# cv3vpl-lab/cylinder-pose-estimation

Hardware: AMD Instinct MI355X
Metric: frames/sec (grid-detect + cylinder fit) on 1920x1200 batch (higher is better)
Workload: dtype f64

## Files before the change

### cylinder-pose-estimation_amd/csrc/masks.hip

```cpp
#include "cpe_dev.h"

namespace cpe {

namespace {

struct W3 { unsigned long long a, b, c; };
template <int K> __device__ __forceinline__ W3 w3_up(const W3 &v, unsigned long long fill)
{
    W3 r;
    r.a = (v.a >> K) | (v.b << (64 - K));
    r.b = (v.b >> K) | (v.c << (64 - K));
    r.c = (v.c >> K) | (fill << (64 - K));
    return r;
}
template <int K> __device__ __forceinline__ W3 w3_down(const W3 &v, unsigned long long fill)
{
    W3 r;
    r.c = (v.c << K) | (v.b >> (64 - K));
    r.b = (v.b << K) | (v.a >> (64 - K));
    r.a = (v.a << K) | (fill >> (64 - K));
    return r;
}
__device__ __forceinline__ W3 w3_and(const W3 &x, const W3 &y) { return W3{x.a & y.a, x.b & y.b, x.c & y.c}; }
__device__ __forceinline__ W3 w3_or(const W3 &x, const W3 &y) { return W3{x.a | y.a, x.b | y.b, x.c | y.c}; }
template <bool IS_AND> __device__ __forceinline__ W3 w3_window20(const W3 &v)
{
    const unsigned long long f = IS_AND ? ~0ull : 0ull;
    auto op = [](const W3 &x, const W3 &y) { return IS_AND ? w3_and(x, y) : w3_or(x, y); };
    const W3 t1 = op(v, w3_up<1>(v, f));
    const W3 t2 = op(t1, w3_up<2>(t1, f));
    const W3 t4 = op(t2, w3_up<4>(t2, f));
    const W3 t8 = op(t4, w3_up<8>(t4, f));
    const W3 t20 = op(t8, w3_up<12>(t4, f));
    return w3_down<10>(t20, f);
}
__device__ __forceinline__ unsigned long long row_valid_word(int j, int w)
{
    const int x0 = j * 64;
    if (j < 0 || x0 >= w) return 0ull;
    return (x0 + 64 <= w) ? ~0ull : ((1ull << (w - x0)) - 1ull);
}
__device__ __forceinline__ unsigned long long bytes_of_bits8(unsigned bits)
{
    unsigned long long v = ((unsigned long long)(bits & 255u) * 0x0101010101010101ull) & 0x8040201008040201ull;
    v = ((v + 0x7f7f7f7f7f7f7f7full) & 0x8080808080808080ull) >> 7;
    return v * 255ull;
}

constexpr int OB_AP = 20;
template <int R>
__global__ __launch_bounds__(256) void k_open20_joints(const uint8_t *__restrict__ bin, int h, int w, int bands,
                                                       uint8_t *__restrict__ hm, uint8_t *__restrict__ vm,
                                                       uint8_t *__restrict__ jm, uint32_t *__restrict__ jbits,
                                                       unsigned long long *__restrict__ hb, unsigned long long *__restrict__ vb)
{
    constexpr int ROWS = R + 2 * OB_AP;
    extern __shared__ unsigned long long s_ob[];
    const int WW = (w + 63) >> 6;
    unsigned long long *buf0 = s_ob, *buf1 = s_ob + (size_t)ROWS * WW, *hbuf = s_ob + (size_t)2 * ROWS * WW;
    const int t = threadIdx.x;
    const int f = blockIdx.x / bands, band = blockIdx.x - f * bands;
    const int y0 = band * R;
    const size_t N = (size_t)h * w;
    const uint8_t *im = bin + f * N;
    const bool al8 = ((w & 7) == 0) && (((size_t)im & 7) == 0);
    {
        uint8_t *pk = reinterpret_cast<uint8_t *>(buf0);
        const int per_row = WW * 8;
        for (int i = t; i < ROWS * per_row; i += 256) {
            const int r = i / per_row, k = i - r * per_row;
            const int y = y0 - OB_AP + r, x0 = k * 8;
            unsigned bits = 255u;
            if (y >= 0 && y < h && x0 < w) {
                const uint8_t *q = im + (size_t)y * w + x0;
                if (al8) {
                    unsigned long long v = *reinterpret_cast<const unsigned long long *>(q);
                    v = (((v & 0x7f7f7f7f7f7f7f7full) + 0x7f7f7f7f7f7f7f7full) | v) & 0x8080808080808080ull;
                    bits = (unsigned)(((v >> 7) * 0x0102040810204080ull) >> 56);
                } else {
                    bits = 0;
                    for (int b = 0; b < 8; b++) bits |= ((x0 + b >= w) || q[b]) ? (1u << b) : 0u;
                }
            }
            pk[i] = (uint8_t)bits;
        }
    }
    __syncthreads();
    for (int i = t; i < R * WW; i += 256) {
        const int tr = i / WW, j = i - tr * WW;
        const unsigned long long *row = buf0 + (size_t)(tr + OB_AP) * WW;
        const W3 x{j > 0 ? row[j - 1] : ~0ull, row[j], j + 1 < WW ? row[j + 1] : ~0ull};
        const W3 v{row_valid_word(j - 1, w), row_valid_word(j, w), row_valid_word(j + 1, w)};
        const W3 e = w3_and(w3_window20<true>(x), v);
        hbuf[i] = w3_window20<false>(e).b & v.b;
    }
    __syncthreads();
    auto pass = [&](const unsigned long long *src, unsigned long long *dst, int step, bool is_and, const unsigned long long *src2) {
        const unsigned long long fill = is_and ? ~0ull : 0ull;
        for (int i = t; i < ROWS * WW; i += 256) {
            const int r = i / WW;
            const unsigned long long p = src[i];
            const unsigned long long q = (r + step < ROWS) ? src2[i + (size_t)step * WW] : fill;
            dst[i] = is_and ? (p & q) : (p | q);
        }
        __syncthreads();
    };
    pass(buf0, buf1, 1, true, buf0);
    pass(buf1, buf0, 2, true, buf1);
    pass(buf0, buf1, 4, true, buf0);
    pass(buf1, buf0, 8, true, buf1);
    for (int i = t; i < ROWS * WW; i += 256) {
        const int r = i / WW;
        const unsigned long long q = (r + 12 < ROWS) ? buf1[i + (size_t)12 * WW] : ~0ull;
        const int y = y0 - 10 + r;
        buf0[i] = (y >= 0 && y < h) ? (buf0[i] & q) : 0ull;
    }
    __syncthreads();
    pass(buf0, buf1, 1, false, buf0);
    pass(buf1, buf0, 2, false, buf1);
    pass(buf0, buf1, 4, false, buf0);
    pass(buf1, buf0, 8, false, buf1);
    {
        const int per_row = WW * 8;
        for (int i = t; hm && i < R * per_row; i += 256) {
            const int tr = i / per_row, k = i - tr * per_row;
            const int y = y0 + tr, x0 = k * 8;
            if (y >= h || x0 >= w) continue;
            const int j = k >> 3, sh = (k & 7) * 8;
            const size_t wi = (size_t)tr * WW + j;
            const unsigned long long d16 = buf0[wi] | ((tr + 12 < ROWS) ? buf1[wi + (size_t)12 * WW] : 0ull);
            const unsigned hb = (unsigned)(hbuf[wi] >> sh) & 255u;
            const unsigned vb = (unsigned)(d16 >> sh) & 255u;
            const size_t o = f * N + (size_t)y * w + x0;
            if (al8 && (((size_t)hm | (size_t)vm | (size_t)jm) & 7) == 0) {
                *reinterpret_cast<unsigned long long *>(hm + o) = bytes_of_bits8(hb);
                *reinterpret_cast<unsigned long long *>(vm + o) = bytes_of_bits8(vb);
                if (jm) *reinterpret_cast<unsigned long long *>(jm + o) = bytes_of_bits8(hb & vb);
            } else {
                for (int b = 0; b < 8 && x0 + b < w; b++) {
                    hm[o + b] = ((hb >> b) & 1u) ? 255 : 0;
                    vm[o + b] = ((vb >> b) & 1u) ? 255 : 0;
                    if (jm) jm[o + b] = (((hb & vb) >> b) & 1u) ? 255 : 0;
                }
            }
        }
        auto plane_word = [&](int tr, int j, bool hsel, bool vsel) {
            const size_t wi = (size_t)tr * WW + j;
            unsigned long long m = ~0ull;
            if (hsel) m &= hbuf[wi];
            if (vsel) m &= buf0[wi] | ((tr + 12 < ROWS) ? buf1[wi + (size_t)12 * WW] : 0ull);
            if (64 * j + 64 > w) m &= (1ull << (w - 64 * j)) - 1ull;
            return m;
        };
        store_plane_band(bit_plane(jbits, f, h, w), h, w, y0, R, t, [&](int tr, int j) { return plane_word(tr, j, true, true); });
        if (hb) {
            const size_t pw = bit_plane_words(h, w);
            store_plane_band(hb + f * pw, h, w, y0, R, t, [&](int tr, int j) { return plane_word(tr, j, true, false); });
            store_plane_band(vb + f * pw, h, w, y0, R, t, [&](int tr, int j) { return plane_word(tr, j, false, true); });
        }
    }
}

constexpr int RB_R = 64, RB_AP = 4, RB_ROWS = RB_R + 2 * RB_AP;
__global__ __launch_bounds__(256) void k_roi_base(const uint8_t *__restrict__ m, const uint8_t *__restrict__ cm,
                                                  const uint8_t *__restrict__ mc, int h, int w, int bands,
                                                  const FrameState *__restrict__ st, uint8_t *__restrict__ roi,
                                                  uint8_t *__restrict__ base, uint8_t *__restrict__ exp,
                                                  uint32_t *__restrict__ bbits, const unsigned long long *__restrict__ mb)
{
    extern __shared__ unsigned long long s_rb[];
    const int WW = (w + 63) >> 6;
    unsigned long long *buf0 = s_rb, *buf1 = s_rb + (size_t)RB_ROWS * WW, *mcb = s_rb + (size_t)2 * RB_ROWS * WW;
    const int t = threadIdx.x;
    const int f = blockIdx.x / bands, band = blockIdx.x - f * bands;
    const int y0 = band * RB_R;
    const size_t N = (size_t)h * w;
    const int *rc = st[f].rect;
    const int rx0 = rc[0], ry0 = rc[1], rx1 = rc[0] + rc[2] - 1, ry1 = rc[1] + rc[3] - 1;
    const bool al8 = ((w & 7) == 0) && ((((size_t)m | (size_t)cm | (size_t)mc | (size_t)roi | (size_t)base | (size_t)exp) & 7) == 0);
    const int per_row = WW * 8;
    auto store8 = [&](uint8_t *dst, size_t o, int x0, unsigned bits) {
        if (al8) *reinterpret_cast<unsigned long long *>(dst + o) = bytes_of_bits8(bits);
        else for (int b = 0; b < 8 && x0 + b < w; b++) dst[o + b] = ((bits >> b) & 1u) ? 255 : 0;
    };
    if (st[f].status == CPE_ST_NO_REGION || y0 > ry1 + RB_AP || y0 + RB_R - 1 < ry0 - RB_AP) {
        for (int i = t; i < RB_R * per_row; i += 256) {
            const int tr = i / per_row, k = i - tr * per_row;
            const int y = y0 + tr, x0 = k * 8;
            if (y >= h || x0 >= w) continue;
            const size_t o = f * N + (size_t)y * w + x0;
            if (roi) store8(roi, o, x0, 0u);
            store8(exp, o, x0, 0u);
            if (base) store8(base, o, x0, 0u);
        }
        store_plane_band(bit_plane(bbits, f, h, w), h, w, y0, RB_R, t, [](int, int) { return 0ull; });
        return;
    }
    {
        uint8_t *pk = reinterpret_cast<uint8_t *>(buf0), *pkc = reinterpret_cast<uint8_t *>(mcb);
        auto nonzero8 = [](unsigned long long v) {
            v = (((v & 0x7f7f7f7f7f7f7f7full) + 0x7f7f7f7f7f7f7f7full) | v) & 0x8080808080808080ull;
            return (unsigned)(((v >> 7) * 0x0102040810204080ull) >> 56);
        };
        const unsigned long long *mbf = mb ? mb + f * bit_plane_words(h, w) : nullptr;
        const int btc = bit_tile_cols(w);
        for (int i = t; i < RB_ROWS * per_row; i += 256) {
            const int r = i / per_row, k = i - r * per_row;
            const int y = y0 - RB_AP + r, x0 = k * 8;
            unsigned bits = 0u, cbits = 0u;
            if (y >= ry0 && y <= ry1 && y >= 0 && y < h && x0 < w && x0 + 7 >= rx0 && x0 <= rx1) {
                const size_t o = f * N + (size_t)y * w + x0;
                const unsigned mbits = mbf ? (unsigned)(mbf[bit_word(btc, y, k >> 3)] >> ((k & 7) * 8)) & 255u : 255u;
                if (al8) {
                    const unsigned long long vc = *reinterpret_cast<const unsigned long long *>(mc + o);
                    unsigned long long v = *reinterpret_cast<const unsigned long long *>(cm + o) & vc;
                    if (!mbf) v &= *reinterpret_cast<const unsigned long long *>(m + o);
                    bits = nonzero8(v) & mbits;
                    cbits = nonzero8(vc);
                } else {
                    for (int b = 0; b < 8 && x0 + b < w; b++) {
                        bits |= (((mbf ? 255 : m[o + b]) & cm[o + b]) & mc[o + b]) ? (1u << b) : 0u;
                        cbits |= mc[o + b] ? (1u << b) : 0u;
                    }
                    bits &= mbits;
                }
            }
            pk[i] = (uint8_t)bits;
            pkc[i] = (uint8_t)cbits;
        }
    }
    __syncthreads();
    auto pass = [&](const unsigned long long *src, unsigned long long *dst, bool dil) {
        const unsigned long long fill = dil ? 0ull : ~0ull;
        for (int i = t; i < RB_ROWS * WW; i += 256) {
            const int r = i / WW, j = i - r * WW;
            unsigned long long acc = fill;
#pragma unroll
            for (int dr = -1; dr <= 1; dr++) {
                const int rr = r + dr, y = y0 - RB_AP + rr;
                unsigned long long hres = fill;
                if (rr >= 0 && rr < RB_ROWS && y >= 0 && y < h) {
                    const unsigned long long *row = src + (size_t)rr * WW;
                    const unsigned long long va = row_valid_word(j - 1, w), vb = row_valid_word(j, w), vc = row_valid_word(j + 1, w);
                    unsigned long long xa = j > 0 ? row[j - 1] : 0ull, xb = row[j], xc = j + 1 < WW ? row[j + 1] : 0ull;
                    if (!dil) { xa |= ~va; xb |= ~vb; xc |= ~vc; }
                    const unsigned long long up = (xb >> 1) | (xc << 63), down = (xb << 1) | (xa >> 63);
                    hres = dil ? (xb | up | down) : (xb & up & down);
                }
                acc = dil ? (acc | hres) : (acc & hres);
            }
            const int y = y0 - RB_AP + r;
            dst[i] = (y >= 0 && y < h) ? (acc & row_valid_word(j, w)) : 0ull;
        }
        __syncthreads();
    };
    auto emit = [&](const unsigned long long *src, uint8_t *dst, uint8_t *dst2, const unsigned long long *and2) {
        for (int i = t; i < RB_R * per_row; i += 256) {
            const int tr = i / per_row, k = i - tr * per_row;
            const int y = y0 + tr, x0 = k * 8;
            if (y >= h || x0 >= w) continue;
            const size_t wi = (size_t)(tr + RB_AP) * WW + (k >> 3);
            const unsigned bits = (unsigned)(src[wi] >> ((k & 7) * 8)) & 255u;
            const size_t o = f * N + (size_t)y * w + x0;
            if (dst) store8(dst, o, x0, bits);
            if (dst2) store8(dst2, o, x0, bits & (unsigned)(and2[wi] >> ((k & 7) * 8)));
        }
    };
    pass(buf0, buf1, false);
    pass(buf1, buf0, true);
    if (roi) emit(buf0, roi, nullptr, nullptr);
    pass(buf0, buf1, true);
    pass(buf1, buf0, false);
    emit(buf0, base, exp, mcb);
    store_plane_band(bit_plane(bbits, f, h, w), h, w, y0, RB_R, t, [&](int tr, int j) { return buf0[(size_t)(tr + RB_AP) * WW + j]; });
}

__global__ __launch_bounds__(64) void k_joint_centroids(const uint32_t *__restrict__ jbits, int h, int w,
                                                        const int *__restrict__ roots, FrameState *__restrict__ st,
                                                        int *__restrict__ jtmp ,
                                                        const unsigned long long *__restrict__ outside, size_t plane_words)
{
    __shared__ unsigned long long s_win[BW_ROWS * 64];
    const int f = blockIdx.y;
    if (st[f].status != CPE_ST_OK) return;
    const int ncomp = min(st[f].n_roots_p, MAXROOTS);
    for (int k = blockIdx.x * 64 + threadIdx.x; k < ncomp; k += gridDim.x * 64) {
        const int root = roots[(size_t)f * MAXROOTS + k];
        if (!comp_is_external(outside + f * plane_words, w, root, 0)) continue;
        BitWin nz{bit_plane(jbits, f, h, w), w, h, s_win + threadIdx.x};
        StatVisitor sv;
        if (!trace_border(nz, root % w, root / w, false, sv, 4 * (w + h) + 65536)) { set_overflow(st[f], OVF_TRACE); continue; }
        sv.finish();
        double m00, m10, m01;
        moments_from_sums(sv.a00, sv.a10, sv.a01, m00, m10, m01);
        if (m00 == 0) continue;
        int cx = (int)(m10 / m00), cy = (int)(m01 / m00);
        atomicAdd(&st[f].n_joints_all, 1);
        const int *r = st[f].rect;
        if (!(r[0] <= cx && cx < r[0] + r[2] && r[1] <= cy && cy < r[1] + r[3])) continue;
        int q = atomicAdd(&st[f].n_joints, 1);
        if (q >= MAXJ) { set_overflow(st[f], OVF_JOINTS); continue; }
        int *o = jtmp + ((size_t)f * MAXJ + q) * 3;
        o[0] = cx; o[1] = cy; o[2] = root;
    }
}

__global__ __launch_bounds__(256) void k_joint_sort(FrameState *__restrict__ st, const int *__restrict__ jtmp,
                                                    int *__restrict__ joints )
{
    const int f = blockIdx.x;
    const int nj = min(st[f].n_joints, MAXJ);
    const int *src = jtmp + (size_t)f * MAXJ * 3;
    int *dst = joints + (size_t)f * MAXJ * 2;
    for (int i = threadIdx.x; i < nj; i += 256) {
        int ki = src[3 * i + 2], rank = 0;
        for (int j = 0; j < nj; j++) rank += (src[3 * j + 2] > ki) ? 1 : 0;
        dst[2 * rank] = src[3 * i];
        dst[2 * rank + 1] = src[3 * i + 1];
    }
    __syncthreads();
    if (threadIdx.x == 0) st[f].n_joints = nj;
}

struct Taps { int k[19]; int r; int shift; };

constexpr int BT_X = 64, BT_Y = 32;
constexpr int B7_R = 3, B7_IH = BT_Y + 2 * B7_R, B7_QW = (BT_X + 8) / 4;
constexpr int B7_LDS_WORDS = B7_IH * BT_X / 2;
static_assert(B7_IH * B7_QW <= B7_LDS_WORDS && BT_X == 64 && BT_Y == 32, "blur_tile's thread maps");
template <int R>
__device__ __forceinline__ void blur_tile(const uint8_t *__restrict__ im, int h, int w, int gx0, int gy0, const Taps &t,
                                          uint8_t *__restrict__ out, uint32_t *s_buf )
{
    static_assert(R == B7_R, "the 7 x 7 tile");
    constexpr int IH = B7_IH, QW = B7_QW, TASKS = IH * (BT_X / 8), PER = (TASKS + 255) / 256;
    const int tid = threadIdx.x;
    const int ax0 = gx0 - 4, ay0 = gy0 - R;
    if (ax0 >= 0 && ax0 + 4 * QW <= w && ay0 >= 0 && ay0 + IH <= h && (w & 3) == 0 && (((size_t)im) & 3) == 0) {
        for (int i = tid; i < IH * QW; i += 256) {
            const int ry = i / QW, q = i - ry * QW;
            s_buf[i] = *reinterpret_cast<const uint32_t *>(im + (size_t)(ay0 + ry) * w + ax0 + 4 * q);
        }
    } else {
        uint8_t *s_in8 = reinterpret_cast<uint8_t *>(s_buf);
        for (int i = tid; i < IH * QW * 4; i += 256) {
            const int ry = i / (4 * QW), b = i - ry * 4 * QW;
            s_in8[i] = im[(size_t)reflect101(ay0 + ry, h) * w + reflect101(ax0 + b, w)];
        }
    }
    __syncthreads();
    uint32_t d[PER][4];
#pragma unroll
    for (int u = 0; u < PER; u++) {
        const int it = tid + 256 * u;
        if (it < TASKS) {
            const int ry = it >> 3, c0 = (it & 7) * 8;
#pragma unroll
// ... 856 lines not shown
    __shared__ uint8_t s_in[IH * IW];
    __shared__ uint16_t s_h[IH * BT_X];
    const int tid = threadIdx.x;
    const int tiles = tiles_x * tiles_y;
    const int f = blockIdx.x / tiles, tt = blockIdx.x - f * tiles;
    const int gx0 = (tt % tiles_x) * BT_X, gy0 = (tt / tiles_x) * BT_Y;
    const size_t N = (size_t)h * w;
    const FrameState &S = st[f];
    if (S.status != CPE_ST_OK) return;
    int half = (int)(S.r0 / 5.0);
    if (half < 3) half = 3;
    if (half > 10) half = half + 5;
    half = max(half, (int)(S.r0 / 4.5));
    const int m = half + 1;
    if (gx0 > S.rect[0] + S.rect[2] + m || gx0 + BT_X < S.rect[0] - m || gy0 > S.rect[1] + S.rect[3] + m || gy0 + BT_Y < S.rect[1] - m)
        return;
    const uint8_t *im = bgr + f * N * 3;
    uint32_t ch[PER][3];
    for (int c = 0; c < 3; c++) {
        for (int i = tid; i < IH * IW; i += 256) {
            int ry = i / IW, rx = i - ry * IW;
            s_in[i] = im[((size_t)reflect101(gy0 - R + ry, h) * w + reflect101(gx0 - R + rx, w)) * 3 + c];
        }
        __syncthreads();
        for (int i = tid; i < IH * BT_X; i += 256) {
            int ry = i / BT_X, rx = i - ry * BT_X;
            const uint8_t *p = &s_in[ry * IW + rx];
            int sacc = 0;
#pragma unroll
            for (int j = 0; j <= 2 * R; j++) sacc += t.k[j] * p[j];
            s_h[i] = (uint16_t)sacc;
        }
        __syncthreads();
#pragma unroll
        for (int q = 0; q < PER; q++) {
            const int i = tid + q * 256;
            int ry = i / BT_X, rx = i - ry * BT_X;
            const uint16_t *p = &s_h[ry * BT_X + rx];
            int sacc = 0;
#pragma unroll
            for (int j = 0; j <= 2 * R; j++) sacc += t.k[j] * (int)p[j * BT_X];
            ch[q][c] = (uint32_t)((sacc + (1 << (t.shift - 1))) >> t.shift);
        }
        __syncthreads();
    }
#pragma unroll
    for (int q = 0; q < PER; q++) {
        const int i = tid + q * 256;
        int ry = i / BT_X, rx = i - ry * BT_X;
        if (gy0 + ry < h && gx0 + rx < w)
            dst[f * N + (size_t)(gy0 + ry) * w + gx0 + rx] = (uint8_t)((ch[q][0] * 3735u + ch[q][1] * 19235u + ch[q][2] * 9798u + 16384u) >> 15);
    }
}

int blur7_bgr(const uint8_t *bgr, int n, int h, int w, const FrameState *st, uint8_t *dst, hipStream_t s)
{
    Taps t7 = {{2, 7, 14, 18, 14, 7, 2}, 3, 12};
    CPE_LAUNCH_BEGIN();
    const int tiles_x = (w + BT_X - 1) / BT_X, tiles_y = (h + BT_Y - 1) / BT_Y;
    CPE_KLAUNCH(k_blur7_bgr, dim3((unsigned)(n * tiles_x * tiles_y)), dim3(256), 0, s, bgr, h, w, tiles_x, tiles_y, t7, st, dst);
    CPE_CHECK_LAUNCH("blur7_bgr");
    return CPE_OK;
}

int blur7_u8(const uint8_t *src, int n, int h, int w, const FrameState *st, uint8_t *dst, hipStream_t s)
{
    Taps t7 = {{2, 7, 14, 18, 14, 7, 2}, 3, 12};
    CPE_LAUNCH_BEGIN();
    const int tiles_x = (w + BT_X - 1) / BT_X, tiles_y = (h + BT_Y - 1) / BT_Y;
    CPE_KLAUNCH((k_blur_fused<3>), dim3((unsigned)(n * tiles_x * tiles_y)), dim3(256), 0, s, src, h, w, tiles_x, tiles_y, t7,
                st, dst);
    CPE_CHECK_LAUNCH("blur7_u8");
    return CPE_OK;
}

int joints_mask_stage(int n, int h, int w, const MaskBuffers &B, FrameState *st, hipStream_t s)
{
    CPE_LAUNCH_BEGIN();
    const bool as_bits = line_masks_as_bits(B, w);
    CPE_CHECK_ARG(!as_bits || 2 * bit_plane_words(h, w) * 8 <= (size_t)h * w, "joints_mask_stage: frame too small for its line-mask planes");
    unsigned long long *hb = as_bits ? line_mask_bits(B, 0, n, h, w) : nullptr, *vb = as_bits ? line_mask_bits(B, 1, n, h, w) : nullptr;
    uint8_t *hm = as_bits && B.skip_debug ? nullptr : B.hmask, *vm = as_bits && B.skip_debug ? nullptr : B.vmask;
    uint8_t *jm = as_bits ? nullptr : B.joints_mask;
    {
        const int WW = (w + 63) / 64;
        const size_t lds64 = (size_t)(2 * (64 + 2 * OB_AP) + 64) * WW * 8, lds32 = (size_t)(2 * (32 + 2 * OB_AP) + 32) * WW * 8;
        CPE_CHECK_HIP(hipFuncSetAttribute(reinterpret_cast<const void *>(&k_open20_joints<64>), hipFuncAttributeMaxDynamicSharedMemorySize, 160 * 1024));
        CPE_CHECK_HIP(hipFuncSetAttribute(reinterpret_cast<const void *>(&k_open20_joints<32>), hipFuncAttributeMaxDynamicSharedMemorySize, 160 * 1024));
        if (lds64 <= 96 * 1024) {
            const int bands = (h + 63) / 64;
            CPE_KLAUNCH(k_open20_joints<64>, dim3((unsigned)(n * bands)), dim3(256), lds64, s, (const uint8_t *)B.binary, h, w, bands,
                        hm, vm, jm, B.jbits, hb, vb);
        } else {
            CPE_CHECK_ARG(lds32 <= 160 * 1024, "joints_mask_stage: frame too wide (%d columns)", w);
            const int bands = (h + 31) / 32;
            CPE_KLAUNCH(k_open20_joints<32>, dim3((unsigned)(n * bands)), dim3(256), lds32, s, (const uint8_t *)B.binary, h, w, bands,
                        hm, vm, jm, B.jbits, hb, vb);
        }
    }
    CPE_CHECK_LAUNCH("joints_mask_stage");
    int rc;
    if ((rc = ccl_components(B.joints_mask, B.jbits, n, h, w, 0, WIN_FRAME, B.lab_p, B.roots_p, ROOTS_JOINTS, st, s)) != CPE_OK) return rc;
    const size_t fl_words = (size_t)h * ((w + 63) / 64);
    return outside_flood(B.joints_mask, n, h, w, st, WIN_FRAME, B.fl_j, B.fl_j + (size_t)n * fl_words, fl_words, s, B.jbits);
}

int spot_stage(const uint8_t *gray, int n, int h, int w, const MaskBuffers &B, FrameState *st, hipStream_t s, int planar)
{
    const size_t total = (size_t)h * w * n;
    int rc;
    CPE_LAUNCH_BEGIN();
    Taps t19 = {{1, 1, 3, 5, 10, 15, 20, 27, 30, 32, 30, 27, 20, 15, 10, 5, 3, 1, 1}, 9, 16};
    {
        const int tiles_x = (w + BT_X - 1) / BT_X, tiles_y = (h + BT_Y - 1) / BT_Y;
        CPE_CHECK_ARG(tiles_x <= 128 && (size_t)tiles_x * tiles_y <= (size_t)MAXROOTS * sizeof(int), "spot_stage: frame too large");
        uint8_t *flags = reinterpret_cast<uint8_t *>(B.roots_s);
        const size_t fstride = (size_t)MAXROOTS * sizeof(int);
        CPE_KLAUNCH(k_spot_scan, dim3((unsigned)(n * tiles_y)), dim3(256), 0, s, gray, h, w, tiles_x, tiles_y, st, flags, fstride);
        CPE_KLAUNCH(k_blur19_spot, dim3((unsigned)(n * tiles_y)), dim3(256), 0, s, gray, h, w, tiles_x, tiles_y, t19,
                    (const uint8_t *)flags, fstride, B.g19);
    }
    if ((rc = ccl_components(B.g19, nullptr, n, h, w, 240, WIN_SPOT, B.lab_s, B.roots_s, ROOTS_SPOT, st, s)) != CPE_OK) return rc;
    CPE_KLAUNCH(k_spot_area, dim3(4, n), dim3(64), 0, s, B.g19, h, w, B.roots_s, st, B.best_s);
    (void)hipMemsetAsync(B.cm, 255, total, s);
    CPE_KLAUNCH(k_spot_ellipse, dim3(n), dim3(64), 0, s, B.g19, n, h, w, B.best_s, st, B.verts, B.cm, planar);
    CPE_CHECK_LAUNCH("spot_stage");
    return CPE_OK;
}

int masks_stage(const uint8_t *gray, int n, int h, int w, const MaskBuffers &B, FrameState *st, hipStream_t s,
                const RegionSide *side, int planar, hipStream_t sj)
{
    int rc;
    CPE_LAUNCH_BEGIN();
    CPE_KLAUNCH(k_masks_reset, dim3((n + 63) / 64), dim3(64), 0, s, st, n);
    const size_t fl_words = bit_plane_words(h, w);
    auto fl_plane = [&](int k) { return bit_plane(B.bits, (size_t)(2 + k) * n, h, w); };
    const bool jside = side && sj != s;
    if (jside) { (void)hipEventRecord(side->clahe_done, s); (void)hipStreamWaitEvent(sj, side->clahe_done, 0); }
    {
        hipStream_t q = jside ? sj : s;
        CPE_KLAUNCH(k_joint_centroids, dim3(frame_waves(n, 16, MAXROOTS / 64), n), dim3(64), 0, q, (const uint32_t *)B.jbits, h, w, B.roots_p, st, B.jtmp,
                    (const unsigned long long *)(B.fl_j + (size_t)n * h * ((w + 63) / 64)), (size_t)h * ((w + 63) / 64));
        CPE_KLAUNCH(k_joint_sort, dim3(n), dim3(256), 0, q, st, B.jtmp, B.joints);
    }
    const int rb_bands = (h + RB_R - 1) / RB_R;
    const size_t rb_lds = (size_t)3 * RB_ROWS * ((w + 63) / 64) * 8;
    CPE_CHECK_ARG(rb_lds <= 160 * 1024, "masks_stage: frame too wide (%d columns)", w);
    CPE_CHECK_HIP(hipFuncSetAttribute(reinterpret_cast<const void *>(&k_roi_base), hipFuncAttributeMaxDynamicSharedMemorySize, 160 * 1024));
    if (side) { (void)hipEventRecord(side->clahe_done, s); (void)hipStreamWaitEvent(side->s, side->clahe_done, 0); }
    for (int which = 0; which < 2; which++) {
        hipStream_t q = (which && side) ? side->s : s;
        const bool as_bits = line_masks_as_bits(B, w);
        const uint8_t *lm = as_bits ? nullptr : (which ? B.vmask : B.hmask);
        const unsigned long long *lmb = as_bits ? line_mask_bits(B, which, n, h, w) : nullptr;
        uint8_t *roi = as_bits && B.skip_debug ? nullptr : (which ? B.roi_v : B.roi_h);
        uint8_t *exp = which ? B.exp_v : B.exp_h;
        int *lab = which ? B.lab_s : B.lab, *roots = which ? B.roots_s : B.roots;
        const RootList list = which ? ROOTS_SPOT : ROOTS_MAIN;
        uint32_t *bits = reinterpret_cast<uint32_t *>(bit_plane(B.bits, which ? (size_t)n : 0, h, w));
        SegRec *segs = B.segs + (size_t)which * n * MAXSEG;
        uint8_t *base = ccl_components_reads_bits(bits, w, lab) ? nullptr : (which ? B.base_v : B.base_h);
        CPE_KLAUNCH(k_roi_base, dim3((unsigned)(n * rb_bands)), dim3(256), rb_lds, q, lm, (const uint8_t *)B.cm, (const uint8_t *)B.mc,
                    h, w, rb_bands, (const FrameState *)st, roi, base, exp, bits, lmb);
        if ((rc = ccl_components(base, bits, n, h, w, 0, WIN_REGION, lab, roots, list, st, q)) != CPE_OK) return rc;
        unsigned long long *fl_bg = fl_plane(2 + 2 * which), *fl_out = fl_plane(3 + 2 * which);
        if ((rc = outside_flood(base, n, h, w, st, WIN_REGION, fl_bg, fl_out, fl_words, q, bits)) != CPE_OK) return rc;
        if (planar) CPE_KLAUNCH((k_seg_trace<8, 700>), dim3(frame_waves(n, 32, 512), n), dim3(64), 0, q, (const uint32_t *)bits, h, w, which, (const int *)roots, list, st, segs, (const unsigned long long *)fl_out, fl_words);
        else CPE_KLAUNCH((k_seg_trace<5, 200>), dim3(frame_waves(n, 32, 512), n), dim3(64), 0, q, (const uint32_t *)bits, h, w, which, (const int *)roots, list, st, segs, (const unsigned long long *)fl_out, fl_words);
        CPE_KLAUNCH(k_seg_global, dim3(n), dim3(256), 0, q, st, which, (const SegRec *)segs);
        if (planar) CPE_KLAUNCH(k_seg_expand<EXP_MAXKS_PLANE>, dim3(frame_waves(n, 32, 256), n), dim3(EXP_NT), 0, q, (const uint32_t *)bits, (const uint8_t *)B.mc, h, w, which, st, (const SegRec *)segs, exp, 201);
        else CPE_KLAUNCH(k_seg_expand<EXP_MAXKS>, dim3(frame_waves(n, 32, 256), n), dim3(EXP_NT), 0, q, (const uint32_t *)bits, (const uint8_t *)B.mc, h, w, which, st, (const SegRec *)segs, exp, 0);
        CPE_CHECK_LAUNCH("masks_stage expand");
        if ((rc = ccl_unions(exp, n, h, w, WIN_REGION, which ? B.lab_v : B.lab_h, st, q)) != CPE_OK) return rc;
    }
    if (side) { (void)hipEventRecord(side->traced, side->s); (void)hipStreamWaitEvent(s, side->traced, 0); }
    return CPE_OK;
}

}
```

Measured before the change: 3946.

## Rewrite morphology kernels as streaming column-strip wavefronts with running counters

Replaces the full-row LDS band kernels for the 20-pixel opening and the ROI/base morphology with 64-thread wavefront kernels. Each lane owns 16 columns inside a strip with halo lanes, uses shuffles for the horizontal windows, and streams down rows. Vertical erosion/dilation comes from bit-sliced running counters or small register delay lines instead of log-step passes through LDS with many block barriers. Output bit planes are staged through a small tile and flushed every 8 rows. This removes large dynamic LDS, most synchronisation and the width limit, at the cost of halo recomputation and a long serial row loop per block.

```diff
diff --git a/cylinder-pose-estimation_amd/csrc/masks.hip b/cylinder-pose-estimation_amd/csrc/masks.hip
--- a/cylinder-pose-estimation_amd/csrc/masks.hip
+++ b/cylinder-pose-estimation_amd/csrc/masks.hip
@@ -4,275 +4,252 @@
 
 namespace {
 
-struct W3 { unsigned long long a, b, c; };
-template <int K> __device__ __forceinline__ W3 w3_up(const W3 &v, unsigned long long fill)
-{
-    W3 r;
-    r.a = (v.a >> K) | (v.b << (64 - K));
-    r.b = (v.b >> K) | (v.c << (64 - K));
-    r.c = (v.c >> K) | (fill << (64 - K));
-    return r;
-}
-template <int K> __device__ __forceinline__ W3 w3_down(const W3 &v, unsigned long long fill)
-{
-    W3 r;
-    r.c = (v.c << K) | (v.b >> (64 - K));
-    r.b = (v.b << K) | (v.a >> (64 - K));
-    r.a = (v.a << K) | (fill >> (64 - K));
-    return r;
-}
-__device__ __forceinline__ W3 w3_and(const W3 &x, const W3 &y) { return W3{x.a & y.a, x.b & y.b, x.c & y.c}; }
-__device__ __forceinline__ W3 w3_or(const W3 &x, const W3 &y) { return W3{x.a | y.a, x.b | y.b, x.c | y.c}; }
-template <bool IS_AND> __device__ __forceinline__ W3 w3_window20(const W3 &v)
+constexpr int BR_HALO = 2, BR_OUT = 64 - 2 * BR_HALO, BR_SPAN = BR_OUT * 16, BR_WORDS = BR_OUT / 4;
+constexpr int BR_TILE = BR_WORDS * 32;
+inline int br_strips(int w) { return (w + BR_SPAN - 1) / BR_SPAN; }
+
+__device__ __forceinline__ unsigned span32(int a, int b)
+{
+    a = max(a, 0); b = min(b, 32);
+    if (a >= b) return 0u;
+    return (b == 32 ? ~0u : (1u << b) - 1u) & ~((1u << a) - 1u);
+}
+__device__ __forceinline__ unsigned long long span64(int a, int b)
+{
+    a = max(a, 0); b = min(b, 64);
+    if (a >= b) return 0ull;
+    return (b == 64 ? ~0ull : (1ull << b) - 1ull) & ~((1ull << a) - 1ull);
+}
+__device__ __forceinline__ unsigned nz4(unsigned v)
+{
+    v = (((v & 0x7f7f7f7fu) + 0x7f7f7f7fu) | v) & 0x80808080u;
+    return ((v >> 7) * 0x10204080u) >> 28;
+}
+__device__ __forceinline__ unsigned nz16(const uint4 &v) { return nz4(v.x) | (nz4(v.y) << 4) | (nz4(v.z) << 8) | (nz4(v.w) << 12); }
+__device__ __forceinline__ unsigned bytes4(unsigned bits)
+{
+    return (((bits & 15u) * 0x00204081u) & 0x01010101u) * 255u;
+}
+__device__ __forceinline__ uint4 load_px16(const uint8_t *p, bool al, int nv)
+{
+    if (al) return *reinterpret_cast<const uint4 *>(p);
+    unsigned v0 = 0, v1 = 0, v2 = 0, v3 = 0;
+#pragma unroll
+    for (int b = 0; b < 4; b++) {
+        if (b < nv) v0 |= (unsigned)p[b] << (8 * b);
+        if (b + 4 < nv) v1 |= (unsigned)p[b + 4] << (8 * b);
+        if (b + 8 < nv) v2 |= (unsigned)p[b + 8] << (8 * b);
+        if (b + 12 < nv) v3 |= (unsigned)p[b + 12] << (8 * b);
+    }
+    return make_uint4(v0, v1, v2, v3);
+}
+__device__ __forceinline__ void store_px16(uint8_t *p, unsigned bits, bool al, int nv)
+{
+    if (al) {
+        *reinterpret_cast<uint4 *>(p) = make_uint4(bytes4(bits), bytes4(bits >> 4), bytes4(bits >> 8), bytes4(bits >> 12));
+        return;
+    }
+#pragma unroll
+    for (int b = 0; b < 16; b++)
+        if (b < nv) p[b] = ((bits >> b) & 1u) ? 255 : 0;
+}
+__device__ __forceinline__ void tile_put(unsigned short *tile, int l, int y, unsigned bits)
+{
+    const int k = l - BR_HALO;
+    if (k >= 0 && k < BR_OUT) tile[(k >> 2) * 32 + (y & 7) * 4 + (k & 3)] = (unsigned short)bits;
+}
+__device__ __forceinline__ void tile_flush(const unsigned short *tile, unsigned long long *plane, int w, int ty, int s, bool last, int l)
+{
+    const int tc = bit_tile_cols(w);
+    unsigned long long *row = plane + (size_t)ty * tc * 8;
+    if (l < BR_OUT) {
+        const int j = s * BR_WORDS + (l >> 2);
+        if (j + 2 < tc) *reinterpret_cast<uint4 *>(row + (size_t)(j + 1) * 8 + (l & 3) * 2) = *reinterpret_cast<const uint4 *>(tile + l * 8);
+    } else {
+        const uint4 z = make_uint4(0, 0, 0, 0);
+        if (s == 0) *reinterpret_cast<uint4 *>(row + (l & 3) * 2) = z;
+        if (last) *reinterpret_cast<uint4 *>(row + (size_t)(tc - 1) * 8 + (l & 3) * 2) = z;
+    }
+}
+
+constexpr int OB_R = 80, OB_RING = 24, OB_LAG = 18;
+template <bool IS_AND> __device__ __forceinline__ unsigned long long window20(unsigned long long v)
 {
     const unsigned long long f = IS_AND ? ~0ull : 0ull;
-    auto op = [](const W3 &x, const W3 &y) { return IS_AND ? w3_and(x, y) : w3_or(x, y); };
-    const W3 t1 = op(v, w3_up<1>(v, f));
-    const W3 t2 = op(t1, w3_up<2>(t1, f));
-    const W3 t4 = op(t2, w3_up<4>(t2, f));
-    const W3 t8 = op(t4, w3_up<8>(t4, f));
-    const W3 t20 = op(t8, w3_up<12>(t4, f));
-    return w3_down<10>(t20, f);
-}
-__device__ __forceinline__ unsigned long long row_valid_word(int j, int w)
-{
-    const int x0 = j * 64;
-    if (j < 0 || x0 >= w) return 0ull;
-    return (x0 + 64 <= w) ? ~0ull : ((1ull << (w - x0)) - 1ull);
-}
-__device__ __forceinline__ unsigned long long bytes_of_bits8(unsigned bits)
-{
-    unsigned long long v = ((unsigned long long)(bits & 255u) * 0x0101010101010101ull) & 0x8040201008040201ull;
-    v = ((v + 0x7f7f7f7f7f7f7f7full) & 0x8080808080808080ull) >> 7;
-    return v * 255ull;
-}
-
-constexpr int OB_AP = 20;
-template <int R>
-__global__ __launch_bounds__(256) void k_open20_joints(const uint8_t *__restrict__ bin, int h, int w, int bands,
-                                                       uint8_t *__restrict__ hm, uint8_t *__restrict__ vm,
-                                                       uint8_t *__restrict__ jm, uint32_t *__restrict__ jbits,
-                                                       unsigned long long *__restrict__ hb, unsigned long long *__restrict__ vb)
-{
-    constexpr int ROWS = R + 2 * OB_AP;
-    extern __shared__ unsigned long long s_ob[];
-    const int WW = (w + 63) >> 6;
-    unsigned long long *buf0 = s_ob, *buf1 = s_ob + (size_t)ROWS * WW, *hbuf = s_ob + (size_t)2 * ROWS * WW;
-    const int t = threadIdx.x;
-    const int f = blockIdx.x / bands, band = blockIdx.x - f * bands;
-    const int y0 = band * R;
+    auto up = [&](unsigned long long x, int k) { return (x >> k) | (f << (64 - k)); };
+    auto op = [](unsigned long long x, unsigned long long y) { return IS_AND ? (x & y) : (x | y); };
+    const unsigned long long t1 = op(v, up(v, 1));
+    const unsigned long long t2 = op(t1, up(t1, 2));
+    const unsigned long long t4 = op(t2, up(t2, 4));
+    const unsigned long long t8 = op(t4, up(t4, 8));
+    const unsigned long long t20 = op(t8, up(t4, 12));
+    return (t20 << 10) | (f >> 54);
+}
+struct Count20 {
+    unsigned b0, b1, b2, b3, b4;
+    __device__ __forceinline__ unsigned full() const { return b4 & (b3 | b2); }
+    __device__ __forceinline__ void step(unsigned keep)
+    {
+        unsigned c = keep & ~full(), t;
+        t = b0 & c; b0 ^= c; c = t;
+        t = b1 & c; b1 ^= c; c = t;
+        t = b2 & c; b2 ^= c; c = t;
+        t = b3 & c; b3 ^= c; c = t;
+        b4 ^= c;
+        b0 &= keep; b1 &= keep; b2 &= keep; b3 &= keep; b4 &= keep;
+    }
+};
+__global__ __launch_bounds__(64) void k_open20_joints(const uint8_t *__restrict__ bin, int h, int w,
+                                                      uint8_t *__restrict__ hm, uint8_t *__restrict__ vm,
+                                                      uint8_t *__restrict__ jm, uint32_t *__restrict__ jbits,
+                                                      unsigned long long *__restrict__ hb, unsigned long long *__restrict__ vb)
+{
+    __shared__ unsigned short s_ring[OB_RING * 64];
+    __shared__ __attribute__((aligned(16))) unsigned short s_tile[3 * BR_TILE];
+    const int l = threadIdx.x, s = blockIdx.x, yb = blockIdx.y * OB_R, f = blockIdx.z;
+    const bool last = s == (int)gridDim.x - 1;
+    const int x0 = (s * BR_OUT + l - BR_HALO) * 16;
+    const bool inx = x0 >= 0 && x0 < w;
+    const bool out = inx && l >= BR_HALO && l < 64 - BR_HALO;
+    const int nv = min(16, w - x0);
+    const unsigned ov = span32(0, nv);
+    const unsigned long long vw = span64(24 - x0, w - x0 + 24);
     const size_t N = (size_t)h * w;
-    const uint8_t *im = bin + f * N;
-    const bool al8 = ((w & 7) == 0) && (((size_t)im & 7) == 0);
-    {
-        uint8_t *pk = reinterpret_cast<uint8_t *>(buf0);
-        const int per_row = WW * 8;
-        for (int i = t; i < ROWS * per_row; i += 256) {
-            const int r = i / per_row, k = i - r * per_row;
-            const int y = y0 - OB_AP + r, x0 = k * 8;
-            unsigned bits = 255u;
-            if (y >= 0 && y < h && x0 < w) {
-                const uint8_t *q = im + (size_t)y * w + x0;
-                if (al8) {
-                    unsigned long long v = *reinterpret_cast<const unsigned long long *>(q);
-                    v = (((v & 0x7f7f7f7f7f7f7f7full) + 0x7f7f7f7f7f7f7f7full) | v) & 0x8080808080808080ull;
-                    bits = (unsigned)(((v >> 7) * 0x0102040810204080ull) >> 56);
-                } else {
-                    bits = 0;
-                    for (int b = 0; b < 8; b++) bits |= ((x0 + b >= w) || q[b]) ? (1u << b) : 0u;
-                }
+    const bool al = ((w & 15) == 0) && ((((size_t)bin | (size_t)hm | (size_t)vm | (size_t)jm) & 15) == 0);
+    const uint8_t *src = bin + f * N + x0;
+    unsigned long long *pj = bit_plane(jbits, f, h, w);
+    const size_t pw = bit_plane_words(h, w);
+    const int y_end = min(yb + OB_R, (h + 7) & ~7);
+    Count20 ce{0u, 0u, 0u, 0u, 0u};
+    Count20 cd{0u, 0u, 0xffffu, 0u, 0xffffu};
+    int wslot = 0, rslot = 0;
+    for (int y = yb - 20; y < y_end + OB_LAG; y++) {
+        const bool iny = y >= 0 && y < h;
+        unsigned xb = 0u;
+        if (iny && inx) xb = nz16(load_px16(src + (size_t)y * w, al, nv));
+        if (y >= yb && y < y_end) {
+            const unsigned p = xb | (__shfl_down(xb, 1) << 16);
+            const unsigned q = __shfl_up(p, 2), r = __shfl_down(p, 2);
+            unsigned long long win = (unsigned long long)((q & 0xffffu) >> 8) | ((unsigned long long)(q >> 16) << 8) |
+                                     ((unsigned long long)xb << 24) | ((unsigned long long)(p >> 16) << 40) |
+                                     ((unsigned long long)(r & 0xffu) << 56);
+            const unsigned long long e = window20<true>(win | ~vw) & vw;
+            const unsigned hres = iny ? (unsigned)((window20<false>(e) & vw) >> 24) & 0xffffu : 0u;
+            s_ring[wslot * 64 + l] = (unsigned short)hres;
+            wslot = wslot + 1 == OB_RING ? 0 : wslot + 1;
+        }
+        ce.step(iny ? xb : 0xffffu);
+        const int ye = y - 9;
+        const unsigned er = (ye >= 0 && ye < h) ? ce.full() : 0u;
+        cd.step(~er & 0xffffu);
+        const int yo = y - OB_LAG;
+        if (yo < yb) continue;
+        unsigned hbits = 0u, vbits = 0u;
+        if (yo < h) {
+            hbits = s_ring[rslot * 64 + l];
+            vbits = ~cd.full() & ov;
+        }
+        rslot = rslot + 1 == OB_RING ? 0 : rslot + 1;
+        if (out && yo < h && hm) {
+            const size_t o = f * N + (size_t)yo * w + x0;
+            store_px16(hm + o, hbits, al, nv);
+            store_px16(vm + o, vbits, al, nv);
+            if (jm) store_px16(jm + o, hbits & vbits, al, nv);
+        }
+        tile_put(s_tile, l, yo, hbits & vbits);
+        if (hb) { tile_put(s_tile + BR_TILE, l, yo, hbits); tile_put(s_tile + 2 * BR_TILE, l, yo, vbits); }
+        if ((yo & 7) == 7) {
+            __syncthreads();
+            tile_flush(s_tile, pj, w, yo >> 3, s, last, l);
+            if (hb) {
+                tile_flush(s_tile + BR_TILE, hb + f * pw, w, yo >> 3, s, last, l);
+                tile_flush(s_tile + 2 * BR_TILE, vb + f * pw, w, yo >> 3, s, last, l);
             }
-            pk[i] = (uint8_t)bits;
-        }
-    }
-    __syncthreads();
-    for (int i = t; i < R * WW; i += 256) {
-        const int tr = i / WW, j = i - tr * WW;
-        const unsigned long long *row = buf0 + (size_t)(tr + OB_AP) * WW;
-        const W3 x{j > 0 ? row[j - 1] : ~0ull, row[j], j + 1 < WW ? row[j + 1] : ~0ull};
-        const W3 v{row_valid_word(j - 1, w), row_valid_word(j, w), row_valid_word(j + 1, w)};
-        const W3 e = w3_and(w3_window20<true>(x), v);
-        hbuf[i] = w3_window20<false>(e).b & v.b;
-    }
-    __syncthreads();
-    auto pass = [&](const unsigned long long *src, unsigned long long *dst, int step, bool is_and, const unsigned long long *src2) {
-        const unsigned long long fill = is_and ? ~0ull : 0ull;
-        for (int i = t; i < ROWS * WW; i += 256) {
-            const int r = i / WW;
-            const unsigned long long p = src[i];
-            const unsigned long long q = (r + step < ROWS) ? src2[i + (size_t)step * WW] : fill;
-            dst[i] = is_and ? (p & q) : (p | q);
-        }
-        __syncthreads();
-    };
-    pass(buf0, buf1, 1, true, buf0);
-    pass(buf1, buf0, 2, true, buf1);
-    pass(buf0, buf1, 4, true, buf0);
-    pass(buf1, buf0, 8, true, buf1);
-    for (int i = t; i < ROWS * WW; i += 256) {
-        const int r = i / WW;
-        const unsigned long long q = (r + 12 < ROWS) ? buf1[i + (size_t)12 * WW] : ~0ull;
-        const int y = y0 - 10 + r;
-        buf0[i] = (y >= 0 && y < h) ? (buf0[i] & q) : 0ull;
-    }
-    __syncthreads();
-    pass(buf0, buf1, 1, false, buf0);
-    pass(buf1, buf0, 2, false, buf1);
-    pass(buf0, buf1, 4, false, buf0);
-    pass(buf1, buf0, 8, false, buf1);
-    {
-        const int per_row = WW * 8;
-        for (int i = t; hm && i < R * per_row; i += 256) {
-            const int tr = i / per_row, k = i - tr * per_row;
-            const int y = y0 + tr, x0 = k * 8;
-            if (y >= h || x0 >= w) continue;
-            const int j = k >> 3, sh = (k & 7) * 8;
-            const size_t wi = (size_t)tr * WW + j;
-            const unsigned long long d16 = buf0[wi] | ((tr + 12 < ROWS) ? buf1[wi + (size_t)12 * WW] : 0ull);
-            const unsigned hb = (unsigned)(hbuf[wi] >> sh) & 255u;
-            const unsigned vb = (unsigned)(d16 >> sh) & 255u;
-            const size_t o = f * N + (size_t)y * w + x0;
-            if (al8 && (((size_t)hm | (size_t)vm | (size_t)jm) & 7) == 0) {
-                *reinterpret_cast<unsigned long long *>(hm + o) = bytes_of_bits8(hb);
-                *reinterpret_cast<unsigned long long *>(vm + o) = bytes_of_bits8(vb);
-                if (jm) *reinterpret_cast<unsigned long long *>(jm + o) = bytes_of_bits8(hb & vb);
-            } else {
-                for (int b = 0; b < 8 && x0 + b < w; b++) {
-                    hm[o + b] = ((hb >> b) & 1u) ? 255 : 0;
-                    vm[o + b] = ((vb >> b) & 1u) ? 255 : 0;
-                    if (jm) jm[o + b] = (((hb & vb) >> b) & 1u) ? 255 : 0;
-                }
-            }
-        }
-        auto plane_word = [&](int tr, int j, bool hsel, bool vsel) {
-            const size_t wi = (size_t)tr * WW + j;
-            unsigned long long m = ~0ull;
-            if (hsel) m &= hbuf[wi];
-            if (vsel) m &= buf0[wi] | ((tr + 12 < ROWS) ? buf1[wi + (size_t)12 * WW] : 0ull);
-            if (64 * j + 64 > w) m &= (1ull << (w - 64 * j)) - 1ull;
-            return m;
-        };
-        store_plane_band(bit_plane(jbits, f, h, w), h, w, y0, R, t, [&](int tr, int j) { return plane_word(tr, j, true, true); });
-        if (hb) {
-            const size_t pw = bit_plane_words(h, w);
-            store_plane_band(hb + f * pw, h, w, y0, R, t, [&](int tr, int j) { return plane_word(tr, j, true, false); });
-            store_plane_band(vb + f * pw, h, w, y0, R, t, [&](int tr, int j) { return plane_word(tr, j, false, true); });
-        }
-    }
-}
-
-constexpr int RB_R = 64, RB_AP = 4, RB_ROWS = RB_R + 2 * RB_AP;
-__global__ __launch_bounds__(256) void k_roi_base(const uint8_t *__restrict__ m, const uint8_t *__restrict__ cm,
-                                                  const uint8_t *__restrict__ mc, int h, int w, int bands,
-                                                  const FrameState *__restrict__ st, uint8_t *__restrict__ roi,
-                                                  uint8_t *__restrict__ base, uint8_t *__restrict__ exp,
-                                                  uint32_t *__restrict__ bbits, const unsigned long long *__restrict__ mb)
-{
-    extern __shared__ unsigned long long s_rb[];
-    const int WW = (w + 63) >> 6;
-    unsigned long long *buf0 = s_rb, *buf1 = s_rb + (size_t)RB_ROWS * WW, *mcb = s_rb + (size_t)2 * RB_ROWS * WW;
-    const int t = threadIdx.x;
-    const int f = blockIdx.x / bands, band = blockIdx.x - f * bands;
-    const int y0 = band * RB_R;
+            __syncthreads();
+        }
+    }
+}
+
+constexpr int RB_R = 40, RB_AP = 4;
+__global__ __launch_bounds__(64) void k_roi_base(const uint8_t *__restrict__ m, const uint8_t *__restrict__ cm,
+                                                 const uint8_t *__restrict__ mc, int h, int w,
+                                                 const FrameState *__restrict__ st, uint8_t *__restrict__ roi,
+                                                 uint8_t *__restrict__ base, uint8_t *__restrict__ exp,
+                                                 uint32_t *__restrict__ bbits, const unsigned long long *__restrict__ mb)
+{
+    __shared__ __attribute__((aligned(16))) unsigned short s_tile[BR_TILE];
+    const int l = threadIdx.x, s = blockIdx.x, yb = blockIdx.y * RB_R, f = blockIdx.z;
+    const bool last = s == (int)gridDim.x - 1;
+    const int c = s * BR_OUT + l - BR_HALO, x0 = c * 16;
+    const bool inx = x0 >= 0 && x0 < w;
+    const bool out = inx && l >= BR_HALO && l < 64 - BR_HALO;
+    const int nv = min(16, w - x0);
+    const unsigned vw = span32(4 - x0, min(24, w - x0 + 4));
     const size_t N = (size_t)h * w;
     const int *rc = st[f].rect;
     const int rx0 = rc[0], ry0 = rc[1], rx1 = rc[0] + rc[2] - 1, ry1 = rc[1] + rc[3] - 1;
-    const bool al8 = ((w & 7) == 0) && ((((size_t)m | (size_t)cm | (size_t)mc | (size_t)roi | (size_t)base | (size_t)exp) & 7) == 0);
-    const int per_row = WW * 8;
-    auto store8 = [&](uint8_t *dst, size_t o, int x0, unsigned bits) {
-        if (al8) *reinterpret_cast<unsigned long long *>(dst + o) = bytes_of_bits8(bits);
-        else for (int b = 0; b < 8 && x0 + b < w; b++) dst[o + b] = ((bits >> b) & 1u) ? 255 : 0;
-    };
-    if (st[f].status == CPE_ST_NO_REGION || y0 > ry1 + RB_AP || y0 + RB_R - 1 < ry0 - RB_AP) {
-        for (int i = t; i < RB_R * per_row; i += 256) {
-            const int tr = i / per_row, k = i - tr * per_row;
-            const int y = y0 + tr, x0 = k * 8;
-            if (y >= h || x0 >= w) continue;
-            const size_t o = f * N + (size_t)y * w + x0;
-            if (roi) store8(roi, o, x0, 0u);
-            store8(exp, o, x0, 0u);
-            if (base) store8(base, o, x0, 0u);
-        }
-        store_plane_band(bit_plane(bbits, f, h, w), h, w, y0, RB_R, t, [](int, int) { return 0ull; });
-        return;
-    }
-    {
-        uint8_t *pk = reinterpret_cast<uint8_t *>(buf0), *pkc = reinterpret_cast<uint8_t *>(mcb);
-        auto nonzero8 = [](unsigned long long v) {
-            v = (((v & 0x7f7f7f7f7f7f7f7full) + 0x7f7f7f7f7f7f7f7full) | v) & 0x8080808080808080ull;
-            return (unsigned)(((v >> 7) * 0x0102040810204080ull) >> 56);
-        };
-        const unsigned long long *mbf = mb ? mb + f * bit_plane_words(h, w) : nullptr;
-        const int btc = bit_tile_cols(w);
-        for (int i = t; i < RB_ROWS * per_row; i += 256) {
-            const int r = i / per_row, k = i - r * per_row;
-            const int y = y0 - RB_AP + r, x0 = k * 8;
-            unsigned bits = 0u, cbits = 0u;
-            if (y >= ry0 && y <= ry1 && y >= 0 && y < h && x0 < w && x0 + 7 >= rx0 && x0 <= rx1) {
+    const bool al = ((w & 15) == 0) && ((((size_t)m | (size_t)cm | (size_t)mc | (size_t)roi | (size_t)base | (size_t)exp) & 15) == 0);
+    const int y_end = min(yb + RB_R, (h + 7) & ~7);
+    const int sx0 = s * BR_SPAN;
+    const bool active = st[f].status != CPE_ST_NO_REGION && yb <= ry1 + RB_AP && yb + RB_R - 1 >= ry0 - RB_AP &&
+                        sx0 <= rx1 + RB_AP && sx0 + BR_SPAN - 1 >= rx0 - RB_AP;
+    const unsigned rm = inx ? span32(rx0 - x0, min(nv, rx1 + 1 - x0)) : 0u;
+    const int ly0 = max(ry0, 0), ly1 = min(ry1, h - 1);
+    const unsigned long long *mbf = mb ? mb + f * bit_plane_words(h, w) : nullptr;
+    const int btc = bit_tile_cols(w);
+    unsigned long long *pb = bit_plane(bbits, f, h, w);
+    unsigned he0 = ~0u, he1 = ~0u, d10 = 0u, d11 = 0u, d20 = 0u, d21 = 0u, e40 = ~0u, e41 = ~0u;
+    unsigned cb0 = 0u, cb1 = 0u, cb2 = 0u, cb3 = 0u;
+    for (int y = active ? yb - RB_AP : yb + RB_AP; y < y_end + RB_AP; y++) {
+        unsigned bs = 0u, rs = 0u, cs = 0u;
+        if (active) {
+            unsigned xb = 0u, cb = 0u;
+            if (rm && y >= ly0 && y <= ly1) {
                 const size_t o = f * N + (size_t)y * w + x0;
-                const unsigned mbits = mbf ? (unsigned)(mbf[bit_word(btc, y, k >> 3)] >> ((k & 7) * 8)) & 255u : 255u;
-                if (al8) {
-                    const unsigned long long vc = *reinterpret_cast<const unsigned long long *>(mc + o);
-                    unsigned long long v = *reinterpret_cast<const unsigned long long *>(cm + o) & vc;
-                    if (!mbf) v &= *reinterpret_cast<const unsigned long long *>(m + o);
-                    bits = nonzero8(v) & mbits;
-                    cbits = nonzero8(vc);
-                } else {
-                    for (int b = 0; b < 8 && x0 + b < w; b++) {
-                        bits |= (((mbf ? 255 : m[o + b]) & cm[o + b]) & mc[o + b]) ? (1u << b) : 0u;
-                        cbits |= mc[o + b] ? (1u << b) : 0u;
-                    }
-                    bits &= mbits;
+                const uint4 vc = load_px16(mc + o, al, nv), va = load_px16(cm + o, al, nv);
+                uint4 v = make_uint4(va.x & vc.x, va.y & vc.y, va.z & vc.z, va.w & vc.w);
+                if (m) {
+                    const uint4 vm = load_px16(m + o, al, nv);
+                    v = make_uint4(v.x & vm.x, v.y & vm.y, v.z & vm.z, v.w & vm.w);
                 }
+                xb = nz16(v) & rm;
+                cb = nz16(vc) & rm;
+                if (mbf) xb &= (unsigned)(mbf[bit_word(btc, y, c >> 2)] >> ((c & 3) * 16));
             }
-            pk[i] = (uint8_t)bits;
-            pkc[i] = (uint8_t)cbits;
-        }
-    }
-    __syncthreads();
-    auto pass = [&](const unsigned long long *src, unsigned long long *dst, bool dil) {
-        const unsigned long long fill = dil ? 0ull : ~0ull;
-        for (int i = t; i < RB_ROWS * WW; i += 256) {
-            const int r = i / WW, j = i - r * WW;
-            unsigned long long acc = fill;
-#pragma unroll
-            for (int dr = -1; dr <= 1; dr++) {
-                const int rr = r + dr, y = y0 - RB_AP + rr;
-                unsigned long long hres = fill;
-                if (rr >= 0 && rr < RB_ROWS && y >= 0 && y < h) {
-                    const unsigned long long *row = src + (size_t)rr * WW;
-                    const unsigned long long va = row_valid_word(j - 1, w), vb = row_valid_word(j, w), vc = row_valid_word(j + 1, w);
-                    unsigned long long xa = j > 0 ? row[j - 1] : 0ull, xb = row[j], xc = j + 1 < WW ? row[j + 1] : 0ull;
-                    if (!dil) { xa |= ~va; xb |= ~vb; xc |= ~vc; }
-                    const unsigned long long up = (xb >> 1) | (xc << 63), down = (xb << 1) | (xa >> 63);
-                    hres = dil ? (xb | up | down) : (xb & up & down);
-                }
-                acc = dil ? (acc | hres) : (acc & hres);
-            }
-            const int y = y0 - RB_AP + r;
-            dst[i] = (y >= 0 && y < h) ? (acc & row_valid_word(j, w)) : 0ull;
-        }
-        __syncthreads();
-    };
-    auto emit = [&](const unsigned long long *src, uint8_t *dst, uint8_t *dst2, const unsigned long long *and2) {
-        for (int i = t; i < RB_R * per_row; i += 256) {
-            const int tr = i / per_row, k = i - tr * per_row;
-            const int y = y0 + tr, x0 = k * 8;
-            if (y >= h || x0 >= w) continue;
-            const size_t wi = (size_t)(tr + RB_AP) * WW + (k >> 3);
-            const unsigned bits = (unsigned)(src[wi] >> ((k & 7) * 8)) & 255u;
-            const size_t o = f * N + (size_t)y * w + x0;
-            if (dst) store8(dst, o, x0, bits);
-            if (dst2) store8(dst2, o, x0, bits & (unsigned)(and2[wi] >> ((k & 7) * 8)));
-        }
-    };
-    pass(buf0, buf1, false);
-    pass(buf1, buf0, true);
-    if (roi) emit(buf0, roi, nullptr, nullptr);
-    pass(buf0, buf1, true);
-    pass(buf1, buf0, false);
-    emit(buf0, base, exp, mcb);
-    store_plane_band(bit_plane(bbits, f, h, w), h, w, y0, RB_R, t, [&](int tr, int j) { return buf0[(size_t)(tr + RB_AP) * WW + j]; });
+            const unsigned win = (xb << 4) | (__shfl_up(xb, 1) >> 12) | ((__shfl_down(xb, 1) & 15u) << 20);
+            auto in_image = [&](int yy) { return yy >= 0 && yy < h; };
+            auto ero3 = [&](unsigned x, int yy) { x |= ~vw; return in_image(yy) ? (x & (x << 1) & (x >> 1)) : ~0u; };
+            auto dil3 = [&](unsigned x) { return x | (x << 1) | (x >> 1); };
+            const unsigned he = ero3(win, y);
+            const unsigned er = in_image(y - 1) ? (he0 & he1 & he & vw) : 0u;
+            he0 = he1; he1 = he;
+            const unsigned d1 = dil3(er);
+            const unsigned ro = in_image(y - 2) ? ((d10 | d11 | d1) & vw) : 0u;
+            d10 = d11; d11 = d1;
+            const unsigned d2 = dil3(ro);
+            const unsigned dd = in_image(y - 3) ? ((d20 | d21 | d2) & vw) : 0u;
+            d20 = d21; d21 = d2;
+            const unsigned e4 = ero3(dd, y - 3);
+            const unsigned ba = in_image(y - 4) ? (e40 & e41 & e4 & vw) : 0u;
+            e40 = e41; e41 = e4;
+            bs = (ba >> 4) & 0xffffu; rs = (ro >> 4) & 0xffffu; cs = cb0;
+            cb0 = cb1; cb1 = cb2; cb2 = cb3; cb3 = cb;
+        }
+        const int yo = y - RB_AP, yr = active ? y - 2 : yo;
+        if (roi && out && yr >= yb && yr < y_end && yr < h) store_px16(roi + f * N + (size_t)yr * w + x0, rs, al, nv);
+        if (yo < yb) continue;
+        if (out && yo < h) {
+            const size_t o = f * N + (size_t)yo * w + x0;
+            store_px16(exp + o, bs & cs, al, nv);
+            if (base) store_px16(base + o, bs, al, nv);
+        }
+        tile_put(s_tile, l, yo, bs);
+        if ((yo & 7) == 7) {
+            __syncthreads();
+            tile_flush(s_tile, pb, w, yo >> 3, s, last, l);
+            __syncthreads();
+        }
+    }
 }
 
 __global__ __launch_bounds__(64) void k_joint_centroids(const uint32_t *__restrict__ jbits, int h, int w,
@@ -1295,22 +1272,9 @@
     unsigned long long *hb = as_bits ? line_mask_bits(B, 0, n, h, w) : nullptr, *vb = as_bits ? line_mask_bits(B, 1, n, h, w) : nullptr;
     uint8_t *hm = as_bits && B.skip_debug ? nullptr : B.hmask, *vm = as_bits && B.skip_debug ? nullptr : B.vmask;
     uint8_t *jm = as_bits ? nullptr : B.joints_mask;
-    {
-        const int WW = (w + 63) / 64;
-        const size_t lds64 = (size_t)(2 * (64 + 2 * OB_AP) + 64) * WW * 8, lds32 = (size_t)(2 * (32 + 2 * OB_AP) + 32) * WW * 8;
-        CPE_CHECK_HIP(hipFuncSetAttribute(reinterpret_cast<const void *>(&k_open20_joints<64>), hipFuncAttributeMaxDynamicSharedMemorySize, 160 * 1024));
-        CPE_CHECK_HIP(hipFuncSetAttribute(reinterpret_cast<const void *>(&k_open20_joints<32>), hipFuncAttributeMaxDynamicSharedMemorySize, 160 * 1024));
-        if (lds64 <= 96 * 1024) {
-            const int bands = (h + 63) / 64;
-            CPE_KLAUNCH(k_open20_joints<64>, dim3((unsigned)(n * bands)), dim3(256), lds64, s, (const uint8_t *)B.binary, h, w, bands,
-                        hm, vm, jm, B.jbits, hb, vb);
-        } else {
-            CPE_CHECK_ARG(lds32 <= 160 * 1024, "joints_mask_stage: frame too wide (%d columns)", w);
-            const int bands = (h + 31) / 32;
-            CPE_KLAUNCH(k_open20_joints<32>, dim3((unsigned)(n * bands)), dim3(256), lds32, s, (const uint8_t *)B.binary, h, w, bands,
-                        hm, vm, jm, B.jbits, hb, vb);
-        }
-    }
+    CPE_CHECK_ARG(n <= 65535 && (h + OB_R - 1) / OB_R <= 65535, "joints_mask_stage: too many frames or rows for one launch");
+    CPE_KLAUNCH(k_open20_joints, dim3((unsigned)br_strips(w), (unsigned)((h + OB_R - 1) / OB_R), (unsigned)n), dim3(64), 0, s,
+                (const uint8_t *)B.binary, h, w, hm, vm, jm, B.jbits, hb, vb);
     CPE_CHECK_LAUNCH("joints_mask_stage");
     int rc;
     if ((rc = ccl_components(B.joints_mask, B.jbits, n, h, w, 0, WIN_FRAME, B.lab_p, B.roots_p, ROOTS_JOINTS, st, s)) != CPE_OK) return rc;
@@ -1357,10 +1321,8 @@
                     (const unsigned long long *)(B.fl_j + (size_t)n * h * ((w + 63) / 64)), (size_t)h * ((w + 63) / 64));
         CPE_KLAUNCH(k_joint_sort, dim3(n), dim3(256), 0, q, st, B.jtmp, B.joints);
     }
-    const int rb_bands = (h + RB_R - 1) / RB_R;
-    const size_t rb_lds = (size_t)3 * RB_ROWS * ((w + 63) / 64) * 8;
-    CPE_CHECK_ARG(rb_lds <= 160 * 1024, "masks_stage: frame too wide (%d columns)", w);
-    CPE_CHECK_HIP(hipFuncSetAttribute(reinterpret_cast<const void *>(&k_roi_base), hipFuncAttributeMaxDynamicSharedMemorySize, 160 * 1024));
+    const dim3 rb_grid((unsigned)br_strips(w), (unsigned)((h + RB_R - 1) / RB_R), (unsigned)n);
+    CPE_CHECK_ARG(n <= 65535 && rb_grid.y <= 65535, "masks_stage: too many frames or rows for one launch");
     if (side) { (void)hipEventRecord(side->clahe_done, s); (void)hipStreamWaitEvent(side->s, side->clahe_done, 0); }
     for (int which = 0; which < 2; which++) {
         hipStream_t q = (which && side) ? side->s : s;
@@ -1374,8 +1336,8 @@
         uint32_t *bits = reinterpret_cast<uint32_t *>(bit_plane(B.bits, which ? (size_t)n : 0, h, w));
         SegRec *segs = B.segs + (size_t)which * n * MAXSEG;
         uint8_t *base = ccl_components_reads_bits(bits, w, lab) ? nullptr : (which ? B.base_v : B.base_h);
-        CPE_KLAUNCH(k_roi_base, dim3((unsigned)(n * rb_bands)), dim3(256), rb_lds, q, lm, (const uint8_t *)B.cm, (const uint8_t *)B.mc,
-                    h, w, rb_bands, (const FrameState *)st, roi, base, exp, bits, lmb);
+        CPE_KLAUNCH(k_roi_base, rb_grid, dim3(64), 0, q, lm, (const uint8_t *)B.cm, (const uint8_t *)B.mc,
+                    h, w, (const FrameState *)st, roi, base, exp, bits, lmb);
         if ((rc = ccl_components(base, bits, n, h, w, 0, WIN_REGION, lab, roots, list, st, q)) != CPE_OK) return rc;
         unsigned long long *fl_bg = fl_plane(2 + 2 * which), *fl_out = fl_plane(3 + 2 * which);
         if ((rc = outside_flood(base, n, h, w, st, WIN_REGION, fl_bg, fl_out, fl_words, q, bits)) != CPE_OK) return rc;
```

Result: faster. 4059, median of 6 (+2.9%).
